# tj12323/GeoPurify

Hardware: AMD Instinct MI355X
Metric: scenes/sec (ScanNet-val shape) + pooled-feature GB/s vs HBM peak (higher is better)
Workload: dtype f32 (student convolutions and pooling: f16 hi/lo split operands, 3 MFMAs per product, fp32 accumulate)

## Files before the change

### geopurify_amd/csrc/error.hip

```cpp
#include <stdarg.h>

#include "gp_common.h"

static thread_local char g_err[512] = "";

extern "C" __attribute__((visibility("hidden"))) void gp_set_error(const char *fmt, ...) {
    va_list ap;
    va_start(ap, fmt);
    vsnprintf(g_err, sizeof(g_err), fmt, ap);
    va_end(ap);
}
extern "C" const char *gp_last_error(void) { return g_err; }
extern "C" int gp_version(void) { return 100; }

int g_gp_knobs[16] = {0, 0, 4, 0, 0, 0, 0, 0, 0, 0, 0, 0, 0, 0, 0, 0};
namespace {
struct KnobRule { int lo, hi; unsigned mask; };
const KnobRule k_rules[16] = {
    {0, -1, 0},
    {0, 4, 0},
    {0, 8, 0},
    {0, 0, 1u | 2u | 4u | 8u | 16u | 32u | 256u | 512u},
    {0, 0, 1u | 2u | 4u | 8u | 16u | 32u | 64u | 128u},
    {0, 1, 0},
    {0, 256, 0},
    {0, 2, 0},
    {0, 0, 1u | 2u | 4u | 8u | 16u},
    {0, 1, 0},
    {0, 64, 0},
    {0, 4, 0},
    {0, 1, 0},
    {0, 64, 0},
    {0, 1, 0},
    {0, 2, 0},
};
}
extern "C" int gp_debug_set(int32_t key, int32_t value) {
    if (key < 1 || key > 15) { gp_set_error("gp_debug_set: no knob %d", key); return GP_EINVAL; }
    const KnobRule &r = k_rules[key];
    const bool ok = r.mask ? (value >= 0 && ((unsigned)value & ~r.mask) == 0u) : (value >= r.lo && value <= r.hi);
    if (!ok || (key == 11 && value != 0 && value != 4) || (key == 7 && value == 1)) {
        gp_set_error("gp_debug_set: value %d is not defined for knob %d", value, key);
        return GP_EINVAL;
    }
    g_gp_knobs[key] = value;
    return GP_OK;
}

void *g_gp_debug_ptr[4] = {nullptr, nullptr, nullptr, nullptr};
size_t g_gp_debug_bytes[4] = {0, 0, 0, 0};
extern "C" int gp_debug_ptr(int32_t key, void *p, size_t bytes) {
    if (key < 0 || key > 3) { gp_set_error("gp_debug_ptr: no buffer %d", key); return GP_EINVAL; }
    if ((p == nullptr) != (bytes == 0)) { gp_set_error("gp_debug_ptr: a buffer comes with its size (and NULL with 0)"); return GP_EINVAL; }
    g_gp_debug_ptr[key] = p;
    g_gp_debug_bytes[key] = bytes;
    return GP_OK;
}
```

### geopurify_amd/csrc/misc.hip

```cpp
#include <cstring>
#include <rocprim/device/device_scan.hpp>

#include "gp_common.h"

namespace {

constexpr int NN_TILE = 1024;

__global__ void __launch_bounds__(256)
nn1_partial_kernel(const float *__restrict__ ref, int64_t n_ref, const float *__restrict__ qry, int64_t n_q,
                   int splits, double *__restrict__ pd, int64_t *__restrict__ pi) {
    __shared__ double sx[NN_TILE], sy[NN_TILE], sz[NN_TILE];
    int64_t q = blockIdx.x * (int64_t)blockDim.x + threadIdx.x;
    int sp = blockIdx.y;
    int64_t per = (n_ref + splits - 1) / splits;
    int64_t r0 = sp * per, r1 = r0 + per < n_ref ? r0 + per : n_ref;
    double qx = 0, qy = 0, qz = 0;
    if (q < n_q) { qx = qry[q * 3]; qy = qry[q * 3 + 1]; qz = qry[q * 3 + 2]; }
    double best = INFINITY;
    int64_t bi = -1;
    for (int64_t t0 = r0; t0 < r1; t0 += NN_TILE) {
        int64_t cnt = r1 - t0 < NN_TILE ? r1 - t0 : NN_TILE;
        __syncthreads();
        for (int j = threadIdx.x; j < cnt; j += 256) {
// ... 274 lines not shown
        if (best <= bound * bound) break;
        if (x0 <= 0 && y0 <= 0 && z0 <= 0 && x1 >= NG - 1 && cy + r >= NG - 1 && cz + r >= NG - 1) break;
    }
    if (lane == 0) nn[q] = bi;
}

__global__ void vis_flags_kernel(const int64_t *__restrict__ mapping, int64_t n, int32_t *__restrict__ f) {
    int64_t i = blockIdx.x * (int64_t)blockDim.x + threadIdx.x;
    if (i < n) f[i] = mapping[i * 3 + 2] != 0 ? 1 : 0;
}
__global__ void vis_compact_kernel(const int64_t *__restrict__ mapping, const int32_t *__restrict__ sc, int64_t n,
                                   int64_t *__restrict__ pt, int64_t *__restrict__ x, int64_t *__restrict__ y,
                                   int64_t *__restrict__ count) {
    int64_t i = blockIdx.x * (int64_t)blockDim.x + threadIdx.x;
    if (i >= n) return;
    bool v = mapping[i * 3 + 2] != 0;
    if (v) { int p = sc[i]; pt[p] = i; x[p] = mapping[i * 3]; y[p] = mapping[i * 3 + 1]; }
    if (i == n - 1) *count = sc[i] + (v ? 1 : 0);
}

size_t scan32_tmp(int64_t n) {
    size_t t = 0;
    (void)rocprim::exclusive_scan(nullptr, t, (int32_t *)nullptr, (int32_t *)nullptr, (int32_t)0, (size_t)n, rocprim::plus<int32_t>(), 0);
    return t;
}

int nn1_splits(int64_t n_ref, int64_t n_q) {
    int64_t qblocks = (n_q + 255) / 256;
    int s = (int)(2048 / (qblocks > 0 ? qblocks : 1));
    if (s < 1) s = 1;
    int64_t maxs = (n_ref + NN_TILE - 1) / NN_TILE;
    if (s > maxs) s = (int)maxs;
    if (s > 64) s = 64;
    return s < 1 ? 1 : s;
}

constexpr int CL_MAXJ = 8;
__device__ __forceinline__ float sum16(float v) {
#pragma unroll
    for (int o = 8; o > 0; o >>= 1) v += __shfl_xor(v, o, 64);
    return v;
}
__global__ void classify16_kernel(const float *__restrict__ feat, int64_t ld, int d, int64_t n, const float *__restrict__ text, int C,
                                  float scale, int64_t *__restrict__ pred, uint8_t *__restrict__ zero_row) {
    const int64_t p = ((blockIdx.x * (int64_t)blockDim.x + threadIdx.x) >> 4);
    const int l = threadIdx.x & 15;
    const bool live = p < n;
    const int nj = d / 64;
    float4 v[CL_MAXJ];
    float ss = 0.f;
#pragma unroll
    for (int j = 0; j < CL_MAXJ; ++j) {
        v[j] = (live && j < nj) ? *reinterpret_cast<const float4 *>(feat + p * ld + (j * 16 + l) * 4) : make_float4(0.f, 0.f, 0.f, 0.f);
        ss += v[j].x * v[j].x + v[j].y * v[j].y + v[j].z * v[j].z + v[j].w * v[j].w;
    }
    ss = sum16(ss);
    const float nrm = fmaxf(sqrtf(ss), 1e-12f);
    float sa = 0.f;
#pragma unroll
    for (int j = 0; j < CL_MAXJ; ++j) {
        v[j].x /= nrm; v[j].y /= nrm; v[j].z /= nrm; v[j].w /= nrm;
        sa += fabsf(v[j].x) + fabsf(v[j].y) + fabsf(v[j].z) + fabsf(v[j].w);
    }
    sa = sum16(sa);
    float bestv = -INFINITY;
    int bestc = 0;
    for (int k = 0; k < C; ++k) {
        float dot = 0.f;
#pragma unroll
        for (int j = 0; j < CL_MAXJ; ++j)
            if (j < nj) {
                const float4 t = *reinterpret_cast<const float4 *>(text + (int64_t)k * d + (j * 16 + l) * 4);
                dot += v[j].x * t.x + v[j].y * t.y + v[j].z * t.z + v[j].w * t.w;
            }
        dot = sum16(dot) * scale;
        if (dot > bestv) { bestv = dot; bestc = k; }
    }
    if (live && l == 0) {
        pred[p] = bestc;
        if (zero_row) zero_row[p] = (sa == 0.f) ? 1 : 0;
    }
}

constexpr int CL_Q = 2;
template <bool GATHER>
__global__ void __launch_bounds__(256)
classify16_lds_kernel(const float *__restrict__ feat, int64_t ld, int d, int64_t n, const float *__restrict__ text, int C,
                      float scale, int64_t *__restrict__ pred, uint8_t *__restrict__ zero_row, const int64_t *__restrict__ index,
                      const int32_t *__restrict__ row_map, float *__restrict__ out, int64_t ld_out) {
    extern __shared__ __align__(16) float cl_text[];
    for (int i = threadIdx.x * 4; i < C * d; i += 256 * 4) *reinterpret_cast<float4 *>(cl_text + i) = *reinterpret_cast<const float4 *>(text + i);
    __syncthreads();
    const int l = threadIdx.x & 15, g = threadIdx.x >> 4;
    const int nj = d / 64;
    for (int64_t base = blockIdx.x * (int64_t)(16 * CL_Q); base < n; base += (int64_t)gridDim.x * (16 * CL_Q)) {
        float4 v[CL_Q][CL_MAXJ];
        float sa[CL_Q], bestv[CL_Q];
        int bestc[CL_Q];
        bool live[CL_Q];
#pragma unroll
        for (int q = 0; q < CL_Q; ++q) {
            const int64_t p = base + g * CL_Q + q;
            live[q] = p < n;
            int64_t src_row = p;
            if constexpr (GATHER) {
                if (live[q]) { src_row = index[p]; if (row_map) src_row = row_map[src_row]; }
            }
            float ss = 0.f;
#pragma unroll
            for (int j = 0; j < CL_MAXJ; ++j) {
                v[q][j] = (live[q] && j < nj) ? *reinterpret_cast<const float4 *>(feat + src_row * ld + (j * 16 + l) * 4) : make_float4(0.f, 0.f, 0.f, 0.f);
                if constexpr (GATHER) {
                    if (live[q] && j < nj) *reinterpret_cast<float4 *>(out + p * ld_out + (j * 16 + l) * 4) = v[q][j];
                }
                ss += v[q][j].x * v[q][j].x + v[q][j].y * v[q][j].y + v[q][j].z * v[q][j].z + v[q][j].w * v[q][j].w;
            }
            ss = sum16(ss);
            const float nrm = fmaxf(sqrtf(ss), 1e-12f);
            float a = 0.f;
#pragma unroll
            for (int j = 0; j < CL_MAXJ; ++j) {
                v[q][j].x /= nrm; v[q][j].y /= nrm; v[q][j].z /= nrm; v[q][j].w /= nrm;
                a += fabsf(v[q][j].x) + fabsf(v[q][j].y) + fabsf(v[q][j].z) + fabsf(v[q][j].w);
            }
            sa[q] = sum16(a);
            bestv[q] = -INFINITY;
            bestc[q] = 0;
        }
        for (int k = 0; k < C; ++k) {
            float dot[CL_Q];
#pragma unroll
            for (int q = 0; q < CL_Q; ++q) dot[q] = 0.f;
#pragma unroll
            for (int j = 0; j < CL_MAXJ; ++j)
                if (j < nj) {
                    const float4 t = *reinterpret_cast<const float4 *>(cl_text + k * d + (j * 16 + l) * 4);
#pragma unroll
                    for (int q = 0; q < CL_Q; ++q) dot[q] += v[q][j].x * t.x + v[q][j].y * t.y + v[q][j].z * t.z + v[q][j].w * t.w;
                }
#pragma unroll
            for (int q = 0; q < CL_Q; ++q) {
                const float dv = sum16(dot[q]) * scale;
                if (dv > bestv[q]) { bestv[q] = dv; bestc[q] = k; }
            }
        }
#pragma unroll
        for (int q = 0; q < CL_Q; ++q)
            if (live[q] && l == 0) {
                const int64_t p = base + g * CL_Q + q;
                pred[p] = bestc[q];
                if (zero_row) zero_row[p] = (sa[q] == 0.f) ? 1 : 0;
            }
    }
}

constexpr int CL_WJ = 16;
__global__ void __launch_bounds__(256)
classify_wave_gather_kernel(const float *__restrict__ feat, int64_t ld, int d, int64_t n, const float *__restrict__ text, int C,
                            float scale, int64_t *__restrict__ pred, uint8_t *__restrict__ zero_row, const int64_t *__restrict__ index,
                            const int32_t *__restrict__ row_map, float *__restrict__ out, int64_t ld_out) {
    extern __shared__ __align__(16) float cl_text[];
    for (int i = threadIdx.x * 4; i < C * d; i += 256 * 4) *reinterpret_cast<float4 *>(cl_text + i) = *reinterpret_cast<const float4 *>(text + i);
    __syncthreads();
    const int lane = threadIdx.x & 63, w = threadIdx.x >> 6;
    const int nj = d / 64;
    for (int64_t base = blockIdx.x * (int64_t)(4 * CL_Q); base < n; base += (int64_t)gridDim.x * (4 * CL_Q)) {
        float u[CL_Q][CL_WJ];
        float sa[CL_Q], bestv[CL_Q];
        int bestc[CL_Q];
        bool live[CL_Q];
#pragma unroll
        for (int q = 0; q < CL_Q; ++q) {
            const int64_t p = base + w * CL_Q + q;
            live[q] = p < n;
            int64_t src_row = 0;
            if (live[q]) { src_row = index[p]; if (row_map) src_row = row_map[src_row]; }
            float ss = 0.f;
#pragma unroll
            for (int j = 0; j < CL_WJ; ++j) {
                u[q][j] = (live[q] && j < nj) ? feat[src_row * ld + j * 64 + lane] : 0.f;
                if (live[q] && j < nj) out[p * ld_out + j * 64 + lane] = u[q][j];
                ss += u[q][j] * u[q][j];
            }
            ss = gp_wave_sum(ss);
            const float nrm = fmaxf(sqrtf(ss), 1e-12f);
            float a = 0.f;
#pragma unroll
            for (int j = 0; j < CL_WJ; ++j) {
                u[q][j] = u[q][j] / nrm;
                a += fabsf(u[q][j]);
            }
            sa[q] = gp_wave_sum(a);
            bestv[q] = -INFINITY;
            bestc[q] = 0;
        }
        for (int k = 0; k < C; ++k) {
            float dot[CL_Q];
#pragma unroll
            for (int q = 0; q < CL_Q; ++q) dot[q] = 0.f;
#pragma unroll
            for (int j = 0; j < CL_WJ; ++j)
                if (j < nj) {
                    const float t = cl_text[k * d + j * 64 + lane];
#pragma unroll
                    for (int q = 0; q < CL_Q; ++q) dot[q] += u[q][j] * t;
                }
#pragma unroll
            for (int q = 0; q < CL_Q; ++q) {
                const float dv = gp_wave_sum(dot[q]) * scale;
                if (dv > bestv[q]) { bestv[q] = dv; bestc[q] = k; }
            }
        }
#pragma unroll
        for (int q = 0; q < CL_Q; ++q)
            if (live[q] && lane == 0) {
                const int64_t p = base + w * CL_Q + q;
                pred[p] = bestc[q];
                if (zero_row) zero_row[p] = (sa[q] == 0.f) ? 1 : 0;
            }
    }
}

__global__ void classify_kernel(const float *__restrict__ feat, int64_t ld, int d, int64_t n,
                                const float *__restrict__ text, int C, float scale, int64_t *__restrict__ pred,
                                uint8_t *__restrict__ zero_row) {
    int64_t p = (blockIdx.x * (int64_t)blockDim.x + threadIdx.x) >> 6;
    if (p >= n) return;
    int lane = gp_lane();
    float ss = 0.f, sa = 0.f;
    for (int c = lane; c < d; c += 64) { float v = feat[p * ld + c]; ss += v * v; }
    ss = gp_wave_sum(ss);
    float nrm = fmaxf(sqrtf(ss), 1e-12f);
    for (int c = lane; c < d; c += 64) sa += fabsf(feat[p * ld + c] / nrm);
    sa = gp_wave_sum(sa);
    float bestv = -INFINITY;
    int bestc = 0;
    for (int k = 0; k < C; ++k) {
        float dot = 0.f;
        for (int c = lane; c < d; c += 64) dot += (feat[p * ld + c] / nrm) * text[(int64_t)k * d + c];
        dot = gp_wave_sum(dot) * scale;
        if (dot > bestv) { bestv = dot; bestc = k; }
    }
    if (lane == 0) {
        pred[p] = bestc;
        if (zero_row) zero_row[p] = (sa == 0.f) ? 1 : 0;
    }
}

__global__ void rows_argmax_kernel(const float *__restrict__ logits, int64_t ld, int C, int64_t n,
                                   const float *__restrict__ feat, int64_t ld_f, int d, int64_t *__restrict__ pred,
                                   uint8_t *__restrict__ zero_row) {
    int64_t p = (blockIdx.x * (int64_t)blockDim.x + threadIdx.x) >> 6;
    if (p >= n) return;
    int lane = gp_lane();
    float bv = -INFINITY;
    int bc = 0x7fffffff;
    for (int c = lane; c < C; c += 64) {
        float v = logits[p * ld + c];
        if (v > bv) { bv = v; bc = c; }
    }
#pragma unroll
    for (int o = 32; o > 0; o >>= 1) {
        float ov = __shfl_xor(bv, o, 64);
        int oc = __shfl_xor(bc, o, 64);
        if (ov > bv || (ov == bv && oc < bc)) { bv = ov; bc = oc; }
    }
    float sa = 0.f;
    if (zero_row && feat) {
        for (int c = lane; c < d; c += 64) sa += fabsf(feat[p * ld_f + c]);
        sa = gp_wave_sum(sa);
    }
    if (lane == 0) {
        pred[p] = bc == 0x7fffffff ? 0 : bc;
        if (zero_row && feat) zero_row[p] = (sa == 0.f) ? 1 : 0;
    }
}

__global__ void iou_hist_kernel(const int64_t *__restrict__ pred, const int64_t *__restrict__ target, int64_t n, int C,
                                const int64_t ig0, const int64_t ig1, const int64_t ig2, const int64_t ig3, int nig,
                                unsigned long long *__restrict__ counts) {
    extern __shared__ unsigned int sh[];
    for (int i = threadIdx.x; i < 3 * C; i += blockDim.x) sh[i] = 0;
    __syncthreads();
    for (int64_t i = blockIdx.x * (int64_t)blockDim.x + threadIdx.x; i < n; i += (int64_t)gridDim.x * blockDim.x) {
        int64_t p = pred[i], t = target[i];
        if ((nig > 0 && t == ig0) || (nig > 1 && t == ig1) || (nig > 2 && t == ig2) || (nig > 3 && t == ig3)) p = t;
        if (p == t && p >= 0 && p < C) atomicAdd(&sh[p], 1u);
        if (p >= 0 && p < C) atomicAdd(&sh[C + p], 1u);
        if (t >= 0 && t < C) atomicAdd(&sh[2 * C + t], 1u);
    }
    __syncthreads();
    for (int i = threadIdx.x; i < 3 * C; i += blockDim.x)
        if (sh[i]) atomicAdd(&counts[i], (unsigned long long)sh[i]);
}

}

extern "C" size_t gp_nn1_workspace_bytes(int64_t n_ref, int64_t n_query) {
    if (n_ref <= 0 || n_query <= 0) return 0;
    int s = nn1_splits(n_ref, n_query);
    GpCarver cv(nullptr, 0);
    cv.take<double>((size_t)s * n_query);
    cv.take<int64_t>((size_t)s * n_query);
    return cv.off;
}

extern "C" int gp_nn1_f64(const float *ref_xyz, int64_t n_ref, const float *query_xyz, int64_t n_query, int64_t *nn,
                          void *workspace, size_t workspace_bytes, void *stream_) {
    GP_CHECK_ARG(ref_xyz && query_xyz && nn && workspace, "gp_nn1_f64: null argument");
    GP_CHECK_ARG(n_ref > 0, "gp_nn1_f64: empty reference set (the reference's KDTree raises here too)");
    if (n_query == 0) return GP_OK;
    int s = nn1_splits(n_ref, n_query);
    GpCarver cv(workspace, workspace_bytes);
    double *pd = cv.take<double>((size_t)s * n_query);
    int64_t *pi = cv.take<int64_t>((size_t)s * n_query);
    if (!cv.ok()) { gp_set_error("gp_nn1_f64: workspace too small (%zu < %zu)", workspace_bytes, cv.off); return GP_ENOMEM; }
    hipStream_t st = gp_stream(stream_);
    dim3 grid((unsigned)((n_query + 255) / 256), (unsigned)s);
    nn1_partial_kernel<<<grid, 256, 0, st>>>(ref_xyz, n_ref, query_xyz, n_query, s, pd, pi);
    nn1_reduce_kernel<<<(int)((n_query + 255) / 256), 256, 0, st>>>(pd, pi, n_query, s, nn);
    GP_CHECK_LAUNCH();
    return GP_OK;
}


extern "C" size_t gp_nn1_masked_workspace_bytes(int64_t n) {
    if (n <= 0) return 0;
    GpCarver cv(nullptr, 0);
    cv.take<int32_t>(n); cv.take<int32_t>(n); cv.take<int32_t>(n); cv.take<int32_t>(n);
    cv.take<float>(3 * n); cv.take<int64_t>(n); cv.take<int64_t>(n); cv.take<int32_t>(64);
    cv.take<char>(scan32_tmp(n > (int64_t)NGMAX * NGMAX * NGMAX + 1 ? n : (int64_t)NGMAX * NGMAX * NGMAX + 1));
    cv.take<float>(8); cv.take<int32_t>(n); cv.take<int32_t>((size_t)NGMAX * NGMAX * NGMAX + 1); cv.take<int32_t>((size_t)NGMAX * NGMAX * NGMAX + 1);
    cv.take<int32_t>((size_t)NGMAX * NGMAX * NGMAX + 1); cv.take<float>(3 * n); cv.take<int64_t>(n);
    cv.take<float>(3 * n); cv.take<int64_t>(n); cv.take<int32_t>(3 * (NG2MAX * NG2MAX * NG2MAX + 1));
    return cv.off;
}

extern "C" int gp_nn1_masked_f64(const float *xyz, int64_t n, const uint8_t *ref_mask, const uint8_t *query_mask,
                                 int64_t *nn, void *workspace, size_t workspace_bytes, void *stream_) {
    GP_CHECK_ARG(xyz && ref_mask && query_mask && nn && workspace, "gp_nn1_masked_f64: null argument");
    GP_CHECK_ARG(n > 0 && n < (1ll << 31), "gp_nn1_masked_f64: n=%lld out of range", (long long)n);
    GpCarver cv(workspace, workspace_bytes);
    int32_t *rf = cv.take<int32_t>(n), *qf = cv.take<int32_t>(n), *rs = cv.take<int32_t>(n), *qs = cv.take<int32_t>(n);
    float *rxyz = cv.take<float>(3 * n);
    int64_t *ridx = cv.take<int64_t>(n), *qidx = cv.take<int64_t>(n);
    int32_t *counts = cv.take<int32_t>(64);
    const int64_t ncell_max = (int64_t)NGMAX * NGMAX * NGMAX;
    int NG = g_gp_knobs[6] > 0 ? g_gp_knobs[6] : 128;
    if (NG > NGMAX) NG = NGMAX;
    const int64_t ncell = (int64_t)NG * NG * NG;
    size_t tb = scan32_tmp(n > ncell_max + 1 ? n : ncell_max + 1);
    char *tmp = cv.take<char>(tb);
    float *bb = cv.take<float>(8);
    int32_t *rcell = cv.take<int32_t>(n);
    int32_t *cell_cnt = cv.take<int32_t>(ncell_max + 1), *cell_start = cv.take<int32_t>(ncell_max + 1), *cursor = cv.take<int32_t>(ncell_max + 1);
    float *sxyz = cv.take<float>(3 * n);
    int64_t *sidx = cv.take<int64_t>(n);
    float *sxyz2 = cv.take<float>(3 * n);
    int64_t *sidx2 = cv.take<int64_t>(n);
    int32_t *cells2 = cv.take<int32_t>(3 * (NG2MAX * NG2MAX * NG2MAX + 1));
    if (!cv.ok()) { gp_set_error("gp_nn1_masked_f64: workspace too small (%zu < %zu)", workspace_bytes, cv.off); return GP_ENOMEM; }
    hipStream_t st = gp_stream(stream_);
    int blocks = (int)((n + 255) / 256);
    mask_flags_kernel<<<blocks, 256, 0, st>>>(ref_mask, query_mask, n, rf, qf);
    size_t t = tb;
    GP_CHECK_HIP(rocprim::exclusive_scan(tmp, t, rf, rs, (int32_t)0, (size_t)n, rocprim::plus<int32_t>(), st));
    t = tb;
    GP_CHECK_HIP(rocprim::exclusive_scan(tmp, t, qf, qs, (int32_t)0, (size_t)n, rocprim::plus<int32_t>(), st));
    mask_compact_kernel<<<blocks, 256, 0, st>>>(xyz, ref_mask, query_mask, rs, qs, n, rxyz, ridx, qidx, counts, nn);
    if (n >= 32768 && !g_gp_knobs[5]) {
        nn_bbox_init_kernel<<<1, 64, 0, st>>>(bb);
        nn_bbox_kernel<<<blocks < 64 ? blocks : 64, 256, 0, st>>>(xyz, n, bb);
        auto bucket = [&](int ng, int32_t *cnt, int32_t *start, int32_t *cur, float *sx, int64_t *si) -> int {
            int64_t nc = (int64_t)ng * ng * ng;
            GP_CHECK_HIP(hipMemsetAsync(cnt, 0, (nc + 1) * sizeof(int32_t), st));
            GP_CHECK_HIP(hipMemsetAsync(cur, 0, (nc + 1) * sizeof(int32_t), st));
            nn_cell_count_kernel<<<blocks, 256, 0, st>>>(rxyz, counts, bb, cnt, rcell, ng);
            size_t tt = tb;
            GP_CHECK_HIP(rocprim::exclusive_scan(tmp, tt, cnt, start, (int32_t)0, (size_t)(nc + 1), rocprim::plus<int32_t>(), st));
            nn_cell_fill_kernel<<<blocks, 256, 0, st>>>(rxyz, ridx, counts, rcell, start, cur, sx, si);
            return GP_OK;
        };
        const bool wave_only = g_gp_knobs[7] != 2;
        int rc = wave_only ? GP_OK : bucket(NG, cell_cnt, cell_start, cursor, sxyz, sidx);
        if (rc) return rc;
        int NG2 = g_gp_knobs[13] > 0 ? g_gp_knobs[13] : 32;
        if (NG2 > NG2MAX) NG2 = NG2MAX;
        const int nc2 = NG2 * NG2 * NG2 + 1;
        rc = bucket(NG2, cells2, cells2 + nc2, cells2 + 2 * nc2, sxyz2, sidx2);
        if (rc) return rc;
        if (wave_only) nn_mark_pending_kernel<<<blocks, 256, 0, st>>>(qidx, counts, nn);
        else nn_grid_query_kernel<<<blocks, 256, 0, st>>>(xyz, sxyz, sidx, cell_start, qidx, counts, bb, nn, NG, 2, 0);
        nn_grid_query_wave_kernel<<<(unsigned)((n * 64 + 255) / 256), 256, 0, st>>>(xyz, sxyz2, sidx2, cells2 + nc2, qidx, counts, bb, nn, NG2);
    } else {
        double *part_d = reinterpret_cast<double *>(cell_cnt);
        int32_t *part_i = reinterpret_cast<int32_t *>(cell_cnt) + 2 * (int64_t)NN_CHUNKS * n;
        static_assert((size_t)NN_CHUNKS * 32768 * 12 <= ((size_t)NGMAX * NGMAX * NGMAX + 1) * 4 * 2, "partials must fit the cell arrays");
        nn1_masked_part_kernel<<<dim3((unsigned)blocks, NN_CHUNKS), 256, 0, st>>>(xyz, rxyz, qidx, counts, part_d, part_i, n);
        nn1_masked_reduce_kernel<<<blocks, 256, 0, st>>>(part_d, part_i, n, ridx, qidx, counts, nn);
    }
    GP_CHECK_LAUNCH();
    return GP_OK;
}

extern "C" size_t gp_visible_lists_workspace_bytes(int64_t n) {
    if (n <= 0) return 0;
    GpCarver cv(nullptr, 0);
    cv.take<int32_t>(n); cv.take<int32_t>(n); cv.take<char>(scan32_tmp(n));
    return cv.off;
}

extern "C" int gp_visible_lists(const int64_t *mapping, int64_t n, int64_t *pt, int64_t *x, int64_t *y,
                                int64_t *count_dev, void *workspace, size_t workspace_bytes, void *stream_) {
    GP_CHECK_ARG(mapping && pt && x && y && count_dev && workspace && n > 0, "gp_visible_lists: null/empty argument");
    GpCarver cv(workspace, workspace_bytes);
    int32_t *f = cv.take<int32_t>(n), *sc = cv.take<int32_t>(n);
    size_t tb = scan32_tmp(n);
    char *tmp = cv.take<char>(tb);
    if (!cv.ok()) { gp_set_error("gp_visible_lists: workspace too small"); return GP_ENOMEM; }
    hipStream_t st = gp_stream(stream_);
    int blocks = (int)((n + 255) / 256);
    vis_flags_kernel<<<blocks, 256, 0, st>>>(mapping, n, f);
    GP_CHECK_HIP(rocprim::exclusive_scan(tmp, tb, f, sc, (int32_t)0, (size_t)n, rocprim::plus<int32_t>(), st));
    vis_compact_kernel<<<blocks, 256, 0, st>>>(mapping, sc, n, pt, x, y, count_dev);
    GP_CHECK_LAUNCH();
    return GP_OK;
}

extern "C" int gp_classify_argmax(const float *feat, int64_t ld, int32_t d, int64_t n, const float *text_norm, int32_t c,
                                  float logit_scale, int64_t *pred, uint8_t *zero_row, void *stream_) {
    GP_CHECK_ARG(feat && text_norm && pred && n > 0 && d > 0 && c > 0, "gp_classify_argmax: null/empty argument");
    const bool fast = d % 64 == 0 && d <= 64 * CL_MAXJ && ld % 4 == 0 && (uintptr_t)feat % 16 == 0 && (uintptr_t)text_norm % 16 == 0;
    const size_t text_bytes = (size_t)c * d * sizeof(float);
    if (fast && text_bytes <= 64 * 1024 && !g_gp_knobs[14]) {
        GP_SMEM_ATTR(classify16_lds_kernel<false>, 64 * 1024);
        const int64_t groups = (n + 16 * CL_Q - 1) / (16 * CL_Q);
        classify16_lds_kernel<false><<<(int)(groups < 2048 ? groups : 2048), 256, text_bytes, gp_stream(stream_)>>>(
            feat, ld, d, n, text_norm, c, logit_scale, pred, zero_row, nullptr, nullptr, nullptr, 0);
    } else if (fast)
        classify16_kernel<<<(int)((n * 16 + 255) / 256), 256, 0, gp_stream(stream_)>>>(feat, ld, d, n, text_norm, c, logit_scale, pred, zero_row);
    else
        classify_kernel<<<(int)((n * 64 + 255) / 256), 256, 0, gp_stream(stream_)>>>(feat, ld, d, n, text_norm, c, logit_scale,
                                                                                   pred, zero_row);
    GP_CHECK_LAUNCH();
    return GP_OK;
}

extern "C" int gp_gather_rows_classify(const float *src, int64_t ld_src, int32_t d, const int64_t *index, int64_t n, const int32_t *row_map,
                                       float *out, int64_t ld_out, const float *text_norm, int32_t c, float logit_scale, int64_t *pred,
                                       uint8_t *zero_row, void *stream_) {
    GP_CHECK_ARG(src && index && out && text_norm && pred && n > 0 && d > 0 && c > 0, "gp_gather_rows_classify: null/empty argument");
    GP_CHECK_ARG(d % 64 == 0 && d <= 64 * CL_WJ && ld_src % 4 == 0 && ld_out % 4 == 0 && ld_out >= d && (uintptr_t)src % 16 == 0 &&
                     (uintptr_t)out % 16 == 0 && (uintptr_t)text_norm % 16 == 0 && (size_t)c * d * sizeof(float) <= 64 * 1024,
                 "gp_gather_rows_classify: d=%d must be a multiple of 64 up to %d, rows 16-byte aligned, c * d * 4 <= 64 KiB (use gp_gather_rows + "
                 "gp_classify_argmax otherwise)", d, 64 * CL_WJ);
    GP_CHECK_ARG(out != src, "gp_gather_rows_classify: out must not alias src");
    if (d <= 64 * CL_MAXJ) {
        GP_SMEM_ATTR(classify16_lds_kernel<true>, 64 * 1024);
        const int64_t groups = (n + 16 * CL_Q - 1) / (16 * CL_Q);
        classify16_lds_kernel<true><<<(int)(groups < 2048 ? groups : 2048), 256, (size_t)c * d * sizeof(float), gp_stream(stream_)>>>(
            src, ld_src, d, n, text_norm, c, logit_scale, pred, zero_row, index, row_map, out, ld_out);
    } else {
        GP_SMEM_ATTR(classify_wave_gather_kernel, 64 * 1024);
        const int64_t groups = (n + 4 * CL_Q - 1) / (4 * CL_Q);
        classify_wave_gather_kernel<<<(int)(groups < 2048 ? groups : 2048), 256, (size_t)c * d * sizeof(float), gp_stream(stream_)>>>(
            src, ld_src, d, n, text_norm, c, logit_scale, pred, zero_row, index, row_map, out, ld_out);
    }
    GP_CHECK_LAUNCH();
    return GP_OK;
}

extern "C" int gp_rows_argmax(const float *logits, int64_t ld, int32_t c, int64_t n, const float *feat, int64_t ld_f,
                              int32_t d, int64_t *pred, uint8_t *zero_row, void *stream_) {
    GP_CHECK_ARG(logits && pred && n > 0 && c > 0, "gp_rows_argmax: null/empty argument");
    rows_argmax_kernel<<<(int)((n * 64 + 255) / 256), 256, 0, gp_stream(stream_)>>>(logits, ld, c, n, feat, ld_f, d, pred, zero_row);
    GP_CHECK_LAUNCH();
    return GP_OK;
}

extern "C" int gp_iou_hist_i64(const int64_t *pred, const int64_t *target, int64_t n, int32_t num_classes,
                               const int64_t *ignore_ids_host, int32_t num_ignore, int64_t *counts, void *stream_) {
    GP_CHECK_ARG(pred && target && counts && n > 0, "gp_iou_hist_i64: null/empty argument");
    GP_CHECK_ARG(num_classes > 0 && num_classes <= 4096, "gp_iou_hist_i64: num_classes=%d out of range", num_classes);
    GP_CHECK_ARG(num_ignore >= 0 && num_ignore <= 4, "gp_iou_hist_i64: at most 4 ignore ids");
    int64_t ig[4] = {0, 0, 0, 0};
    for (int i = 0; i < num_ignore; ++i) ig[i] = ignore_ids_host[i];
    int blocks = (int)((n + 255) / 256);
    if (blocks > 1024) blocks = 1024;
    iou_hist_kernel<<<blocks, 256, 3 * num_classes * sizeof(unsigned int), gp_stream(stream_)>>>(
        pred, target, n, num_classes, ig[0], ig[1], ig[2], ig[3], num_ignore,
        reinterpret_cast<unsigned long long *>(counts));
    GP_CHECK_LAUNCH();
    return GP_OK;
}
```

### geopurify_amd/ops.py

```python
import ctypes

import numpy as np
import torch

from . import _lib
from ._lib import check


def _ptr(t):
    return ctypes.c_void_p(t.data_ptr()) if t is not None else None


def _stream():
    return ctypes.c_void_p(torch.cuda.current_stream().cuda_stream)


def _ws(nbytes, device):
    return torch.empty(max(int(nbytes), 256), dtype=torch.uint8, device=device)


def _chk(t, dtype, name):
    if t.dtype != dtype or not t.is_cuda or not t.is_contiguous():
        raise ValueError(f"{name}: expected contiguous CUDA {dtype}, got {t.dtype} cuda={t.is_cuda} contig={t.is_contiguous()}")
    return t
# ... 96 lines not shown
    def status(self):
        return int(self.buf[36:40].view(torch.int32).item())


def grid_build(coords_sorted, origin=None, extent=None):
    lib = _lib.load()
    _chk(coords_sorted, torch.int32, "coords")
    nv = coords_sorted.shape[0]
    if origin is None or extent is None:
        lo = coords_sorted.amin(0)
        hi = coords_sorted.amax(0)
        lohi = torch.stack([lo, hi]).cpu().tolist()
        origin = lohi[0]
        extent = [lohi[1][a] - lohi[0][a] + 1 for a in range(3)]
    o = (ctypes.c_int32 * 3)(*[int(v) for v in origin])
    e = (ctypes.c_int32 * 3)(*[int(v) for v in extent])
    nbytes = lib.gp_grid_bytes(nv, e)
    if nbytes == 0:
        raise _lib.GeoPurifyHipError("gp_grid_bytes: invalid extent")
    buf = _ws(nbytes, coords_sorted.device)
    check(lib.gp_grid_build(_ptr(coords_sorted), nv, o, e, _ptr(buf), buf.numel(), _stream()), "gp_grid_build")
    return Grid(buf, list(origin), list(extent), nv)


def kernel_map_build(grid, coords_sorted):
    lib = _lib.load()
    nv = coords_sorted.shape[0]
    nm = torch.empty((27, nv), dtype=torch.int32, device=coords_sorted.device)
    check(lib.gp_kernel_map_build(_ptr(grid.buf), _ptr(coords_sorted), nv, _ptr(nm), _stream()), "gp_kernel_map_build")
    return nm


def coords_order_batched(coords_b):
    lib = _lib.load()
    _chk(coords_b, torch.int32, "coords")
    if coords_b.dim() != 2 or coords_b.shape[1] != 4:
        raise ValueError(f"coords_order_batched: expected [nv, 4], got {list(coords_b.shape)}")
    nv = coords_b.shape[0]
    dev = coords_b.device
    ws = _ws(lib.gp_coords_order_batched_workspace_bytes(nv), dev)
    perm = torch.empty(nv, dtype=torch.int32, device=dev)
    rank = torch.empty(nv, dtype=torch.int32, device=dev)
    keys = torch.empty(nv, dtype=torch.int64, device=dev)
    status = torch.empty(3, dtype=torch.int32, device=dev)
    check(lib.gp_coords_order_batched(_ptr(coords_b), nv, _ptr(perm), _ptr(rank), _ptr(keys), _ptr(status), _ptr(ws), ws.numel(),
                                      _stream()), "gp_coords_order_batched")
    return perm, rank, keys, status


def kernel_map_sorted(keys_sorted):
    lib = _lib.load()
    _chk(keys_sorted, torch.int64, "keys")
    nv = keys_sorted.shape[0]
    nm = torch.empty((27, nv), dtype=torch.int32, device=keys_sorted.device)
    check(lib.gp_kernel_map_sorted(_ptr(keys_sorted), nv, _ptr(nm), _stream()), "gp_kernel_map_sorted")
    return nm


class QuantizedIndex:

    def __init__(self, n, nv, coordinates, unique_index, inverse, order, seg_start, bad_batch, bad_axes):
        self.n, self.nv, self.coordinates, self.unique_index, self.inverse = n, nv, coordinates, unique_index, inverse
        self.order, self.seg_start, self.bad_batch, self.bad_axes = order, seg_start, bad_batch, bad_axes
        self.counts = seg_start[1:] - seg_start[:-1]


QUANTIZE_OUTPUTS = {"vox_coords": (torch.int32, lambda n: (n, 4)), "unique_index": (torch.int64, lambda n: (n,)),
                    "inverse": (torch.int64, lambda n: (n,)), "order": (torch.int64, lambda n: (n,)),
                    "seg_start": (torch.int64, lambda n: (n + 1,)), "status": (torch.int32, lambda n: (3,))}


def quantize_batched(coords_b, buffers=None):
    lib = _lib.load()
    _chk(coords_b, torch.int32, "coords")
    if coords_b.dim() != 2 or coords_b.shape[1] != 4:
        raise ValueError(f"quantize_batched: expected [n, 4], got {list(coords_b.shape)}")
    n = coords_b.shape[0]
    if not 0 < n < 2 ** 31:
        raise ValueError(f"quantize_batched: n={n} out of range (1 .. 2^31 - 1)")
    dev = coords_b.device
    b = {}
    for name, (dtype, shape) in QUANTIZE_OUTPUTS.items():
        t = (buffers or {}).get(name)
        if t is None:
            t = torch.empty(shape(n), dtype=dtype, device=dev)
        elif _chk(t, dtype, name).shape != shape(n) or t.device != dev:
            raise ValueError(f"quantize_batched: buffer {name} must be {list(shape(n))} on {dev}, got {list(t.shape)} on {t.device}")
        b[name] = t
    ws = _ws(lib.gp_quantize_batched_workspace_bytes(n), dev)
    check(lib.gp_quantize_batched(_ptr(coords_b), n, _ptr(b["vox_coords"]), _ptr(b["unique_index"]), _ptr(b["inverse"]),
                                  _ptr(b["order"]), _ptr(b["seg_start"]), _ptr(b["status"]), _ptr(ws), ws.numel(), _stream()),
          "gp_quantize_batched")
    nv, bad_batch, bad_axes = readback(b["status"])
    return QuantizedIndex(n, nv, b["vox_coords"][:nv], b["unique_index"][:nv], b["inverse"], b["order"], b["seg_start"][:nv + 1],
                     bad_batch, bad_axes)


SEGMENT_LABEL_RULES = {"first": 0, "differ": 1, "count": 2}


def segment_labels(labels, q, ignore_label, rule, out=None):
    lib = _lib.load()
    if rule not in SEGMENT_LABEL_RULES:
        raise ValueError(f"segment_labels: rule={rule!r}, expected one of {sorted(SEGMENT_LABEL_RULES)}")
    _chk(labels, torch.int64, "labels")
    if labels.dim() != 1 or labels.shape[0] != q.n:
        raise ValueError(f"segment_labels: expected labels [{q.n}], got {list(labels.shape)}")
    if labels.device != q.order.device:
        raise ValueError(f"segment_labels: labels on {labels.device}, the quantisation on {q.order.device}")
    if out is None:
        out = torch.empty(q.nv, dtype=torch.int64, device=labels.device)
    elif _chk(out, torch.int64, "out").shape != (q.nv,) or out.device != labels.device:
        raise ValueError(f"segment_labels: expected out [{q.nv}], got {list(out.shape)}")
    check(lib.gp_segment_labels(_ptr(labels), q.n, _ptr(q.order), _ptr(q.seg_start), _ptr(q.unique_index), q.nv, int(ignore_label),
                                SEGMENT_LABEL_RULES[rule], _ptr(out), _stream()), "gp_segment_labels")
    return out


def scatter_mean_csr(src, d, order, seg_start, nv, out, col0=0, row_map=None):
    lib = _lib.load()
    _chk(src, torch.float32, "src")
    check(lib.gp_scatter_mean_csr(_ptr(src), src.stride(0), int(d), _ptr(order), _ptr(seg_start), int(nv),
                                  _ptr(row_map), _ptr(out), out.stride(0), int(col0), _stream()),
          "gp_scatter_mean_csr")
    return out


def voxel_rows_operands(f, d, geo, dg, order, seg_start, nv, cin_pad, row_map=None, want_scale=True):
    lib = _lib.load()
    _chk(f, torch.float32, "f")
    _chk(geo, torch.float32, "geo")
    dev = f.device
    X = torch.empty((nv, cin_pad), dtype=torch.float32, device=dev)
    rows = torch.empty((nv, 2 * cin_pad), dtype=torch.float16, device=dev)
    rinv = torch.empty(nv, dtype=torch.float32, device=dev)
    sc = torch.empty(2, dtype=torch.float32, device=dev) if want_scale else None
    ws = _ws(256, dev) if want_scale else None
    check(lib.gp_voxel_rows_operands(_ptr(f), f.stride(0), int(d), _ptr(geo), geo.stride(0), int(dg), _ptr(order), _ptr(seg_start), int(nv),
                                     _ptr(row_map), _ptr(X), X.stride(0), int(cin_pad), _ptr(rows), rows.stride(0), _ptr(rinv), _ptr(sc),
                                     _ptr(ws), ws.numel() if ws is not None else 0, _stream()), "gp_voxel_rows_operands")
    return X, (rows, None, rinv), sc


def gather_rows(src, d, index, out=None, row_map=None):
    lib = _lib.load()
    n = index.shape[0]
    if out is None:
        out = torch.empty((n, d), dtype=torch.float32, device=src.device)
    check(lib.gp_gather_rows(_ptr(src), src.stride(0), int(d), _ptr(index), n, _ptr(row_map), _ptr(out),
                             out.stride(0), _stream()), "gp_gather_rows")
    return out


def gather_rows_classify(src, d, index, text_norm, logit_scale, row_map=None):
    lib = _lib.load()
    n = index.shape[0]
    out = torch.empty((n, d), dtype=torch.float32, device=src.device)
    pred = torch.empty(n, dtype=torch.int64, device=src.device)
    zero = torch.empty(n, dtype=torch.uint8, device=src.device)
    check(lib.gp_gather_rows_classify(_ptr(src), src.stride(0), int(d), _ptr(index), n, _ptr(row_map), _ptr(out), out.stride(0),
                                      _ptr(text_norm), int(text_norm.shape[0]), float(logit_scale), _ptr(pred), _ptr(zero), _stream()),
          "gp_gather_rows_classify")
    return out, pred, zero


def can_gather_rows_classify(d, num_classes):
    return d % 64 == 0 and d <= 1024 and num_classes * d * 4 <= 64 * 1024


def pool_cs_width_ok(d):
    return d % 256 == 0 and 256 <= d <= 1024


def sparse_conv(x, nbr_map, w, scale=None, shift=None, residual=None, relu=False, out=None):
    lib = _lib.load()
    nv = x.shape[0]
    if w.dim() == 3:
        kv, cin, cout = w.shape
    else:
        kv, (cin, cout) = 1, w.shape
    _chk(w, torch.float32, "w")
    if out is None:
        out = torch.empty((nv, cout), dtype=torch.float32, device=x.device)
    check(lib.gp_sparse_conv(_ptr(x), x.stride(0), _ptr(nbr_map) if kv > 1 else None, nv, _ptr(w), int(kv),
                             int(cin), int(cout), _ptr(scale), _ptr(shift), _ptr(residual),
                             residual.stride(0) if residual is not None else 0, int(bool(relu)), _ptr(out),
                             out.stride(0), _stream()), "gp_sparse_conv")
    return out


class ConvPairs:

    def __init__(self, pair_in, pair_pos, seg_off, tile_start, nseg, num_pairs, nv):
        self.pair_in, self.pair_pos, self.pair_off, self.tile_start = pair_in, pair_pos, seg_off, tile_start
        self.nseg, self.num_pairs, self.nv = nseg, num_pairs, nv
        self.partial = None
        self.num_chunks, self.chunk_row_off, self.chunk_tile_off, self.chunk_pair_off = 0, None, None, None

    def _set_chunks(self, rows, tiles, pairs):
        n = len(rows) - 1
        self.num_chunks = n
        self.chunk_row_off = (ctypes.c_int32 * (n + 1))(*rows)
        self.chunk_tile_off = (ctypes.c_int32 * (n + 1))(*tiles)
        self.chunk_pair_off = (ctypes.c_int32 * (n + 1))(*pairs)
        self.max_chunk_pairs = max(pairs[i + 1] - pairs[i] for i in range(n))

    def regroup(self, g):
        g = max(1, min(int(g), max(self.num_chunks, 1)))
        cp = ConvPairs(self.pair_in, self.pair_pos, self.pair_off, self.tile_start, self.nseg, self.num_pairs, self.nv)
        cp.tile_desc = self.tile_desc
        n = self.num_chunks
        idx = list(range(0, n, g)) + [n]
        ro, po, to = list(self.chunk_row_off), list(self.chunk_pair_off), list(self.chunk_tile_off)
        cp._set_chunks([ro[i] for i in idx], [to[i] for i in idx], [po[i] for i in idx])
        return cp


CONV_TARGET_TILES = None


def conv_pairs_build(nbr_map, chunk_rows="balanced", col_tiles=2):
    lib = _lib.load()
    kv, nv = nbr_map.shape
    dev = nbr_map.device
    if isinstance(chunk_rows, str):
        if chunk_rows != "balanced":
            raise ValueError(f"conv_pairs_build: chunk_rows={chunk_rows!r}")
    if isinstance(chunk_rows, str):
        granule = 256
        max_chunks = (nv + granule - 1) // granule
        plan = torch.empty(max_chunks + 2, dtype=torch.int32, device=dev)
        ws = _ws(lib.gp_conv_chunk_plan_workspace_bytes(nv, granule), dev)
        target = CONV_TARGET_TILES or 3 * torch.cuda.get_device_properties(dev).multi_processor_count - 16
        check(lib.gp_conv_chunk_plan(_ptr(nbr_map), nv, kv, granule, int(col_tiles), int(target), max_chunks, _ptr(plan),
                                     _ptr(plan[max_chunks + 1:]), _ptr(ws), ws.numel(), _stream()), "gp_conv_chunk_plan")
        host = readback(plan)
        nchunks = host[max_chunks + 1]
        rows = host[:nchunks + 1]
        row_off = plan[:nchunks + 1]
    else:
        ch = nv if chunk_rows is None else max(int(chunk_rows), 256)
        rows = list(range(0, nv, ch)) + [nv]
        nchunks = len(rows) - 1
        row_off = torch.tensor(rows, dtype=torch.int32, device=dev)
    nseg = nchunks * kv
    ws = _ws(lib.gp_conv_pairs_workspace_bytes(nv, kv), dev)
    pair_in = torch.empty(kv * nv, dtype=torch.int32, device=dev)
    pair_pos = torch.empty((kv, nv), dtype=torch.int32, device=dev)
    seg_off = torch.empty(nseg + 1, dtype=torch.int32, device=dev)
    tile_start = torch.empty(nseg + 1, dtype=torch.int32, device=dev)
    tile_desc = torch.empty(((kv * nv) // 256 + nseg + 1, 4), dtype=torch.int32, device=dev)
    check(lib.gp_conv_pairs_build(_ptr(nbr_map), nv, kv, nchunks, _ptr(row_off), _ptr(pair_in), _ptr(pair_pos), _ptr(seg_off),
                                  _ptr(tile_start), _ptr(tile_desc), _ptr(ws), ws.numel(), _stream()), "gp_conv_pairs_build")
    bounds = readback(torch.stack([seg_off[::kv], tile_start[::kv]]))
    num_pairs = bounds[0][-1]
    cp = ConvPairs(pair_in, pair_pos, seg_off, tile_start, nseg, num_pairs, nv)
    cp.tile_desc = tile_desc
    cp._set_chunks(rows, bounds[1], bounds[0])
    return cp


def conv_weights_split(w, scale_pow2, blocked=None, transpose_flip=False):
    lib = _lib.load()
    kv, cin, cout = w.shape
    if transpose_flip:
        if cout % 32 == 0 and cin % 256 == 0 and blocked is not False:
            hi = torch.empty((kv, cin // 256, cout // 32, 256, 32), dtype=torch.float16, device=w.device)
            lo = torch.empty_like(hi)
            check(lib.gp_conv_weights_split_blocked(_ptr(w), kv, cout, cin, float(scale_pow2), _ptr(hi), _ptr(lo), 1, _stream()),
                  "gp_conv_weights_split_blocked")
            return hi, lo
        return conv_weights_split(w.flip(0).transpose(1, 2).contiguous(), scale_pow2, blocked)
    if blocked is None:
        blocked = cin % 32 == 0 and cout % 256 == 0
    if blocked:
        hi = torch.empty((kv, cout // 256, cin // 32, 256, 32), dtype=torch.float16, device=w.device)
        lo = torch.empty_like(hi)
        check(lib.gp_conv_weights_split_blocked(_ptr(w), kv, cin, cout, float(scale_pow2), _ptr(hi), _ptr(lo), 0, _stream()),
              "gp_conv_weights_split_blocked")
        return hi, lo
    hi = torch.empty((kv, cout, cin), dtype=torch.float16, device=w.device)
    lo = torch.empty((kv, cout, cin), dtype=torch.float16, device=w.device)
    check(lib.gp_conv_weights_split(_ptr(w), kv, cin, cout, float(scale_pow2), _ptr(hi), _ptr(lo), _stream()),
          "gp_conv_weights_split")
    return hi, lo


def conv_weights_shape(w_hi):
    if w_hi.dim() == 5:
        return int(w_hi.shape[0]), int(w_hi.shape[1]) * 256, int(w_hi.shape[2]) * 32
    return tuple(int(v) for v in w_hi.shape)


def split_f16(x, d=None, scale=None, per_row=False, interleaved=False, dst_row=None, extra_zero_rows=0):
    lib = _lib.load()
    d = x.shape[1] if d is None else d
    if interleaved:
        assert per_row and d % 32 == 0, "interleaved rows are the row-scaled operand of the convolution"
        rows = torch.empty((x.shape[0], 2 * d), dtype=torch.float16, device=x.device)
        rinv = torch.empty(x.shape[0], dtype=torch.float32, device=x.device)
        check(lib.gp_split_f16_scaled(_ptr(x), x.stride(0), int(d), x.shape[0], _ptr(rows), None, rows.stride(0), None, _ptr(rinv),
                                      _ptr(dst_row), _stream()), "gp_split_f16_scaled")
        return rows, None, rinv
    hi = torch.empty((x.shape[0] + extra_zero_rows, d), dtype=torch.float16, device=x.device)
    lo = torch.empty((x.shape[0] + extra_zero_rows, d), dtype=torch.float16, device=x.device)
    if extra_zero_rows:
        hi[x.shape[0]:].zero_()
        lo[x.shape[0]:].zero_()
# ... 1433 lines not shown
```

Baseline: 47.50.

## Add software-pipelined gather-classify kernel with DPP reductions and resident grid

Adds a new gather+classify kernel templated on feature width. It prefetches the gathered rows and index entries two and three iterations ahead so that load latency overlaps the dot-product work. It replaces the 16-lane shuffle reductions with DPP-based sums and sizes the grid to the resident occupancy per CU, caching that size across calls. The old path stays reachable through knob 14 = 2 as a reference. The cost is more registers per thread from the prefetch buffers and template instantiations for each width.

After: 47.58, median of 3. No clear change (+0.2%).

```diff
diff --git a/geopurify_amd/csrc/error.hip b/geopurify_amd/csrc/error.hip
--- a/geopurify_amd/csrc/error.hip
+++ b/geopurify_amd/csrc/error.hip
@@ -31,7 +31,7 @@
     {0, 4, 0},
     {0, 1, 0},
     {0, 64, 0},
-    {0, 1, 0},
+    {0, 2, 0},
     {0, 2, 0},
 };
 }
diff --git a/geopurify_amd/csrc/misc.hip b/geopurify_amd/csrc/misc.hip
--- a/geopurify_amd/csrc/misc.hip
+++ b/geopurify_amd/csrc/misc.hip
@@ -450,6 +450,121 @@
                 if (zero_row) zero_row[p] = (sa[q] == 0.f) ? 1 : 0;
             }
     }
+}
+
+template <int CTRL>
+__device__ __forceinline__ float dpp16(float v) {
+    return __int_as_float(__builtin_amdgcn_update_dpp(0, __float_as_int(v), CTRL, 0xf, 0xf, false));
+}
+__device__ __forceinline__ float sum16_dpp(float v) {
+    v += dpp16<0x128>(v);
+    v += dpp16<0x1B>(dpp16<0x141>(v));
+    v += dpp16<0x4E>(v);
+    v += dpp16<0xB1>(v);
+    return v;
+}
+
+template <int NJ, bool MAP>
+__global__ void __launch_bounds__(256)
+gather_classify16_kernel(const float *__restrict__ feat, int64_t ld, int64_t n, const float *__restrict__ text, int C, float scale,
+                         int64_t *__restrict__ pred, uint8_t *__restrict__ zero_row, const int64_t *__restrict__ index,
+                         const int32_t *__restrict__ row_map, float *__restrict__ out, int64_t ld_out) {
+    extern __shared__ __align__(16) float cl_text[];
+    constexpr int d = NJ * 64;
+    const int l = threadIdx.x & 15, g = threadIdx.x >> 4;
+    const int64_t step = (int64_t)gridDim.x * (16 * CL_Q), last = n - 1;
+    int64_t base = blockIdx.x * (int64_t)(16 * CL_Q) + g * CL_Q;
+    int64_t rn[CL_Q], i2[CL_Q];
+    float4 nx[CL_Q][NJ];
+#pragma unroll
+    for (int q = 0; q < CL_Q; ++q) {
+        const int64_t p0 = base + q, p1 = p0 + step, p2 = p1 + step;
+        int64_t r0 = index[p0 < last ? p0 : last];
+        rn[q] = index[p1 < last ? p1 : last];
+        i2[q] = index[p2 < last ? p2 : last];
+        if constexpr (MAP) { r0 = row_map[r0]; rn[q] = row_map[rn[q]]; }
+#pragma unroll
+        for (int j = 0; j < NJ; ++j) nx[q][j] = *reinterpret_cast<const float4 *>(feat + r0 * ld + (j * 16 + l) * 4);
+    }
+    for (int i = threadIdx.x * 4; i < C * d; i += 256 * 4) *reinterpret_cast<float4 *>(cl_text + i) = *reinterpret_cast<const float4 *>(text + i);
+    __syncthreads();
+    for (; base - g * CL_Q < n; base += step) {
+        float4 v[CL_Q][NJ];
+        float sa[CL_Q], bestv[CL_Q];
+        int bestc[CL_Q];
+#pragma unroll
+        for (int q = 0; q < CL_Q; ++q) {
+            const int64_t p3 = base + q + 3 * step;
+            const int64_t r1 = rn[q];
+#pragma unroll
+            for (int j = 0; j < NJ; ++j) {
+                v[q][j] = nx[q][j];
+                nx[q][j] = *reinterpret_cast<const float4 *>(feat + r1 * ld + (j * 16 + l) * 4);
+            }
+            if constexpr (MAP) rn[q] = row_map[i2[q]]; else rn[q] = i2[q];
+            i2[q] = index[p3 < last ? p3 : last];
+        }
+#pragma unroll
+        for (int q = 0; q < CL_Q; ++q) {
+            const int64_t p = base + q;
+            if (p < n) {
+#pragma unroll
+                for (int j = 0; j < NJ; ++j) *reinterpret_cast<float4 *>(out + p * ld_out + (j * 16 + l) * 4) = v[q][j];
+            }
+        }
+#pragma unroll
+        for (int q = 0; q < CL_Q; ++q) {
+            float ss = 0.f;
+#pragma unroll
+            for (int j = 0; j < NJ; ++j) ss += v[q][j].x * v[q][j].x + v[q][j].y * v[q][j].y + v[q][j].z * v[q][j].z + v[q][j].w * v[q][j].w;
+            ss = sum16_dpp(ss);
+            const float nrm = fmaxf(sqrtf(ss), 1e-12f);
+            float a = 0.f;
+#pragma unroll
+            for (int j = 0; j < NJ; ++j) {
+                v[q][j].x /= nrm; v[q][j].y /= nrm; v[q][j].z /= nrm; v[q][j].w /= nrm;
+                a += fabsf(v[q][j].x) + fabsf(v[q][j].y) + fabsf(v[q][j].z) + fabsf(v[q][j].w);
+            }
+            sa[q] = sum16_dpp(a);
+            bestv[q] = -INFINITY;
+            bestc[q] = 0;
+        }
+        for (int k = 0; k < C; ++k) {
+            float dot[CL_Q];
+#pragma unroll
+            for (int q = 0; q < CL_Q; ++q) dot[q] = 0.f;
+#pragma unroll
+            for (int j = 0; j < NJ; ++j) {
+                const float4 t = *reinterpret_cast<const float4 *>(cl_text + k * d + (j * 16 + l) * 4);
+#pragma unroll
+                for (int q = 0; q < CL_Q; ++q) dot[q] += v[q][j].x * t.x + v[q][j].y * t.y + v[q][j].z * t.z + v[q][j].w * t.w;
+            }
+#pragma unroll
+            for (int q = 0; q < CL_Q; ++q) {
+                const float dv = sum16_dpp(dot[q]) * scale;
+                if (dv > bestv[q]) { bestv[q] = dv; bestc[q] = k; }
+            }
+        }
+#pragma unroll
+        for (int q = 0; q < CL_Q; ++q)
+            if (base + q < n && l == 0) {
+                pred[base + q] = bestc[q];
+                if (zero_row) zero_row[base + q] = (sa[q] == 0.f) ? 1 : 0;
+            }
+    }
+}
+
+template <int NJ>
+int gather_classify16_resident(int &per_cu, size_t text_bytes) {
+    GP_SMEM_ATTR((gather_classify16_kernel<NJ, true>), 64 * 1024);
+    GP_SMEM_ATTR((gather_classify16_kernel<NJ, false>), 64 * 1024);
+    GP_CHECK_HIP(hipOccupancyMaxActiveBlocksPerMultiprocessor(&per_cu, gather_classify16_kernel<NJ, true>, 256, text_bytes));
+    return GP_OK;
+}
+template <int NJ, typename... A>
+void gather_classify16_launch(int grid, size_t text_bytes, hipStream_t st, bool map, A... a) {
+    if (map) gather_classify16_kernel<NJ, true><<<grid, 256, text_bytes, st>>>(a...);
+    else gather_classify16_kernel<NJ, false><<<grid, 256, text_bytes, st>>>(a...);
 }
 
 constexpr int CL_WJ = 16;
@@ -753,7 +868,46 @@
                  "gp_gather_rows_classify: d=%d must be a multiple of 64 up to %d, rows 16-byte aligned, c * d * 4 <= 64 KiB (use gp_gather_rows + "
                  "gp_classify_argmax otherwise)", d, 64 * CL_WJ);
     GP_CHECK_ARG(out != src, "gp_gather_rows_classify: out must not alias src");
-    if (d <= 64 * CL_MAXJ) {
+    const size_t text_bytes = (size_t)c * d * sizeof(float);
+    if (d <= 64 * CL_MAXJ && g_gp_knobs[14] != 2) {
+        static std::atomic<uint64_t> s_resident{0};
+        const int nj = d / 64;
+        const uint64_t shape = ((uint64_t)d << 48) | ((uint64_t)text_bytes << 24);
+        uint64_t res = s_resident.load(std::memory_order_relaxed);
+        if ((res & ~(uint64_t)0xffffff) != shape || (res & 0xffffff) == 0) {
+            int per_cu = 0, rc = GP_OK;
+            switch (nj) {
+            case 1: rc = gather_classify16_resident<1>(per_cu, text_bytes); break;
+            case 2: rc = gather_classify16_resident<2>(per_cu, text_bytes); break;
+            case 3: rc = gather_classify16_resident<3>(per_cu, text_bytes); break;
+            case 4: rc = gather_classify16_resident<4>(per_cu, text_bytes); break;
+            case 5: rc = gather_classify16_resident<5>(per_cu, text_bytes); break;
+            case 6: rc = gather_classify16_resident<6>(per_cu, text_bytes); break;
+            case 7: rc = gather_classify16_resident<7>(per_cu, text_bytes); break;
+            default: rc = gather_classify16_resident<8>(per_cu, text_bytes); break;
+            }
+            if (rc != GP_OK) return rc;
+            const int n_cu = gp_cu_count();
+            GP_CHECK_ARG(per_cu > 0 && n_cu > 0 && (int64_t)per_cu * n_cu < (1 << 24), "gp_gather_rows_classify: cannot size the resident grid");
+            res = shape | (uint64_t)(per_cu * n_cu);
+            s_resident.store(res, std::memory_order_relaxed);
+        }
+        const int64_t groups = (n + 16 * CL_Q - 1) / (16 * CL_Q), resident = (int64_t)(res & 0xffffff);
+        const int grid = (int)(groups < resident ? groups : resident);
+        hipStream_t st = gp_stream(stream_);
+#define GP_GC16(NJ) gather_classify16_launch<NJ>(grid, text_bytes, st, row_map != nullptr, src, ld_src, n, text_norm, c, logit_scale, pred, zero_row, index, row_map, out, ld_out)
+        switch (nj) {
+        case 1: GP_GC16(1); break;
+        case 2: GP_GC16(2); break;
+        case 3: GP_GC16(3); break;
+        case 4: GP_GC16(4); break;
+        case 5: GP_GC16(5); break;
+        case 6: GP_GC16(6); break;
+        case 7: GP_GC16(7); break;
+        default: GP_GC16(8); break;
+        }
+#undef GP_GC16
+    } else if (d <= 64 * CL_MAXJ) {
         GP_SMEM_ATTR(classify16_lds_kernel<true>, 64 * 1024);
         const int64_t groups = (n + 16 * CL_Q - 1) / (16 * CL_Q);
         classify16_lds_kernel<true><<<(int)(groups < 2048 ? groups : 2048), 256, (size_t)c * d * sizeof(float), gp_stream(stream_)>>>(
diff --git a/geopurify_amd/ops.py b/geopurify_amd/ops.py
--- a/geopurify_amd/ops.py
+++ b/geopurify_amd/ops.py
@@ -272,8 +272,14 @@
     return out
 
 
-def gather_rows_classify(src, d, index, text_norm, logit_scale, row_map=None):
-    lib = _lib.load()
+def gather_rows_classify(src, d, index, text_norm, logit_scale, row_map=None, reference=False):
+    lib = _lib.load()
+    if reference:
+        check(lib.gp_debug_set(14, 2), "gp_debug_set")
+        try:
+            return gather_rows_classify(src, d, index, text_norm, logit_scale, row_map=row_map)
+        finally:
+            check(lib.gp_debug_set(14, 0), "gp_debug_set")
     n = index.shape[0]
     out = torch.empty((n, d), dtype=torch.float32, device=src.device)
     pred = torch.empty(n, dtype=torch.int64, device=src.device)
```
